# flydog-sdr/FlyDog_SDR_GPS

Measured on NVIDIA B200. Metric: acquisition cells/sec (PRN x Doppler x code-phase), higher is better.
Workload: dtype f32

## Files before the change

flydog_sdr_gps_b200/_build.py:

```python
import os
import shutil
import subprocess

HERE = os.path.dirname(os.path.abspath(__file__))
CSRC = os.path.join(HERE, "csrc")
LIB = os.path.join(CSRC, "libacq_b200.so")
CU_SOURCES = ["acq_kernels.cu", "acq_api.cu", "acq_microbench.cu"]
CPP_SOURCES = ["search_dropin.cpp"]
HEADERS = ["acq_fft.cuh", "acq_geom.h", "acq_kernels.cuh", "e1b_codes.inc", os.path.join("..", "..", "include", "search_dropin.h"),
           os.path.join("..", "..", "include", "acq_b200.h")]

NVCC_FLAGS = ["-gencode", "arch=compute_100a,code=sm_100a", "-lineinfo", "-O3", "-std=c++17",
              "-Xcompiler", "-fPIC", "-shared"]


def _nvcc():
    for cand in (shutil.which("nvcc"), "/usr/local/cuda/bin/nvcc"):
        if cand and os.path.exists(cand):
            return cand
    raise RuntimeError("nvcc not found: cannot build libacq_b200.so")


def needs_build():
    if not os.path.exists(LIB):
        return True
    t = os.path.getmtime(LIB)
    deps = [os.path.join(CSRC, f) for f in CU_SOURCES + CPP_SOURCES + HEADERS]
    return any(os.path.exists(d) and os.path.getmtime(d) > t for d in deps)


def build(force=False, verbose=False, defines=(), out=None):
    if out is None and not force and not needs_build():
        return LIB
    lib = out or LIB
    srcs = [os.path.join(CSRC, f) for f in CU_SOURCES + CPP_SOURCES if os.path.exists(os.path.join(CSRC, f))]
    cmd = [_nvcc()] + NVCC_FLAGS + ["-D" + d for d in defines] + (["-Xptxas", "-v"] if verbose else []) + ["-o", lib + ".tmp"] + srcs
    res = subprocess.run(cmd, capture_output=True, text=True)
    if res.returncode != 0:
        raise RuntimeError("nvcc failed:\n%s\n%s" % (" ".join(cmd), res.stderr[-4000:]))
    os.replace(lib + ".tmp", lib)
    if verbose:
        print(res.stderr)
    return lib


VARIANTS = {
    "l1_multi_tw": ["ACQ_VARIANT_L1_MULTI_TW"],
    "l1_mst": ["ACQ_VARIANT_L1_MST"],
    "l1_cta": ["ACQ_FORCE_L1_CTA=1"],
    "l1_dr_all": ["ACQ_DR_MIN_TILES_PER_SM=0"],
    "l1_dr12": ["ACQ_DR_MIN_TILES_PER_SM=12"],
    "l1_nocr": ["ACQ_L1_CR=0"],
    "l1_sp": ["ACQ_VARIANT_L1_SP"],
    "l1_st": ["ACQ_VARIANT_L1_ST"],
    "l1_ldg": ["ACQ_VARIANT_L1_LDG"],
    "l1_x3": ["ACQ_VARIANT_L1_X3"],
    "l1_x3t": ["ACQ_VARIANT_L1_X3", "ACQ_X3_TMA_D"],
    "e1b_ldg": ["ACQ_VARIANT_E1B_LDG", "ACQ_FORCE_E1B_KERNEL=1"],
    "e1b_cta": ["ACQ_FORCE_E1B_KERNEL=1"],
    "e1b_cluster": ["ACQ_FORCE_E1B_KERNEL=2"],
    "trace": ["ACQ_TRACE"],
    "pdl0": ["ACQ_FORCE_PDL=0"],
    "pdl1": ["ACQ_FORCE_PDL=1"],
    "zcin": ["ACQ_ZC_INPUT=1"],
    "static_tiles": ["ACQ_DYN_MIN_ROUNDS=1000000000"],
    "dyn_tiles": ["ACQ_DYN_MIN_ROUNDS=0"],
    "carve0": ["ACQ_CARVEOUT_MAX=0"],
    "argin0": ["ACQ_ARG_INPUT=0"],
    "devrec": ["ACQ_HOST_RECORDS=0"],
}


def variant_path(name):
    return os.path.join(CSRC, "variants", "libacq_b200_%s.so" % name)


def build_variant(name, force=False):
    path = variant_path(name)
    deps = [os.path.join(CSRC, f) for f in CU_SOURCES + CPP_SOURCES + HEADERS + ["acq_variants.cuh"]]
    fresh = os.path.exists(path) and all(os.path.getmtime(d) <= os.path.getmtime(path) for d in deps if os.path.exists(d))
    if fresh and not force:
        return path
    os.makedirs(os.path.dirname(path), exist_ok=True)
    return build(defines=VARIANTS[name], out=path)


if __name__ == "__main__":
    print(build(force=True, verbose=True))
```

flydog_sdr_gps_b200/csrc/acq_fft.cuh:

```cuda
#pragma once

#include <cuda_runtime.h>
#include <stdint.h>

#include "acq_geom.h"

namespace acq {

__constant__ float2 c_cC[4][16];

__device__ __forceinline__ float2 bc(float s) { return make_float2(s, s); }
__device__ __forceinline__ float2 jmul(float2 a) { return make_float2(-a.y, a.x); }
__device__ __forceinline__ float2 cneg(float2 a) { return make_float2(-a.x, -a.y); }
__device__ __forceinline__ float2 cadd(float2 a, float2 b) { return __fadd2_rn(a, b); }
__device__ __forceinline__ float2 csub(float2 a, float2 b) { return __fadd2_rn(a, cneg(b)); }
__device__ __forceinline__ float2 cadd_jb(float2 a, float2 b) { return __fadd2_rn(a, jmul(b)); }
__device__ __forceinline__ float2 csub_jb(float2 a, float2 b) { return __fadd2_rn(a, cneg(jmul(b))); }
__device__ __forceinline__ float2 cmul(float2 a, float2 w)
{
    return __ffma2_rn(jmul(a), bc(w.y), __fmul2_rn(a, bc(w.x)));
}
__device__ __forceinline__ float2 cfma(float2 a, float2 w, float2 c)
{
    return __ffma2_rn(jmul(a), bc(w.y), __ffma2_rn(a, bc(w.x), c));
// ... 422 lines not shown
    tmem_wait_ld();
    b = TW_AT(15);
    __syncwarp();
    if constexpr (SWZ128) {
        {
            const uint32_t wb = smem_u32(row + c);
            asm volatile("st.shared.v2.f32 [%0], {%1, %2};" ::"r"(wb), "f"(x[r16(0)].x), "f"(x[r16(0)].y) : "memory");
#pragma unroll
            for (int i = 0; i < 15; i++) {
                const int n1 = i + 1;
                const float2 v = cmul(x[r16(n1)], TW_AT(i));
                asm volatile("st.shared.v2.f32 [%0], {%1, %2};" ::"r"((wb ^ (16u * (n1 & 7))) + 128u * n1), "f"(v.x), "f"(v.y) : "memory");
            }
        }
        __syncwarp();
        {
            const uint32_t rb = smem_u32(row + 16 * c + 2 * (c & 7));
#pragma unroll
            for (int j = 0; j < 8; j++)
                asm volatile("ld.shared.v4.f32 {%0, %1, %2, %3}, [%4];"
                             : "=f"(x[2 * j].x), "=f"(x[2 * j].y), "=f"(x[2 * j + 1].x), "=f"(x[2 * j + 1].y)
                             : "r"(rb ^ (16u * j))
                             : "memory");
        }
    } else {
        {
            const uint32_t wb = smem_u32(row + c);
            asm volatile("st.shared.v2.f32 [%0], {%1, %2};" ::"r"(wb), "f"(x[r16(0)].x), "f"(x[r16(0)].y) : "memory");
#pragma unroll
            for (int i = 0; i < 15; i++) {
                const int n1 = i + 1;
                const float2 v = cmul(x[r16(n1)], TW_AT(i));
                asm volatile("st.shared.v2.f32 [%0], {%1, %2};" ::"r"((wb ^ (8u * n1)) + 128u * n1), "f"(v.x), "f"(v.y) : "memory");
            }
        }
        __syncwarp();
        {
            const uint32_t rb = smem_u32(row + 17 * c);
#pragma unroll
            for (int cc = 0; cc < 16; cc++)
                asm volatile("ld.shared.v2.f32 {%0, %1}, [%2];" : "=f"(x[cc].x), "=f"(x[cc].y) : "r"(rb ^ (8u * cc)) : "memory");
        }
    }
    radix16_inv(x);
}
#undef TW_AT

template <bool SWZ128, class PostBarrier>
__device__ __forceinline__ void subfft4096_inv4(float2 (&x)[16], const int k2, float2 &b, float2 *S1b, const int t,
                                                const uint32_t tw_taddr, PostBarrier &&post_barrier)
{
    subfft4096_inv4<SWZ128>(x, k2, b, S1b, t, tw_taddr, [] { __syncthreads(); }, post_barrier);
}

__device__ __forceinline__ void tmem_ld1(uint32_t taddr, float2 &v)
{
    asm volatile("tcgen05.ld.sync.aligned.32x32b.x2.b32 {%0,%1}, [%2];" : "=f"(v.x), "=f"(v.y) : "r"(taddr) : "memory");
}
__device__ __forceinline__ void tmem_st1(uint32_t taddr, const float2 v)
{
    asm volatile("tcgen05.st.sync.aligned.32x32b.x2.b32 [%0], {%1,%2};" ::"r"(taddr), "f"(v.x), "f"(v.y) : "memory");
}

constexpr uint32_t kSwz = ACQ_SWZ128 ? 16u : 8u;
constexpr int kSwzMask = ACQ_SWZ128 ? 7 : 15;

struct BaseFromTmem {
    uint32_t taddr;
    float2 v;
    __device__ __forceinline__ void issue(int k2) { tmem_ld1(taddr + 2 * ((k2 + 1) & 3), v); }
    __device__ __forceinline__ float2 get()
    {
        tmem_wait_ld();
        return v;
    }
};
struct BaseFromGlobal {
    const float2 *bases;
    float2 v;
    __device__ __forceinline__ void issue(int k2) { v = __ldg(bases + 256 * ((k2 + 1) & 3)); }
    __device__ __forceinline__ float2 get() { return v; }
};

template <class BaseSrc, class TeamBarrier, class PostBarrier>
__device__ __forceinline__ void subfft4096_inv4s(float2 (&x)[16], const int k2, float2 &b, float2 *S1b, const int t,
                                                 const float2 *T2s, BaseSrc base_src, TeamBarrier &&team_barrier,
                                                 PostBarrier &&post_barrier)
{
    radix16_inv(x);
    stage_a_store<256>(x, b, S1b + t);
#ifndef ACQ_E1B_TW15
#define ACQ_E1B_TW15 1
#endif
    float2 tw[ACQ_E1B_TW15 ? 15 : 8];
    const float2 *twp = T2s + k2 * (15 * 16) + (t & 15);
#pragma unroll
    for (int i = 0; i < (ACQ_E1B_TW15 ? 15 : 8); i++) tw[i] = twp[i * 16];
    base_src.issue(k2);
    team_barrier();
    post_barrier();
    float2 *row = S1b + (t >> 4) * 256;
    const int c = t & 15;
    {
        const float2 *src = row + c;
#pragma unroll
        for (int bb = 0; bb < 16; bb++) x[bb] = src[16 * bb];
    }
    radix16_inv(x);
    b = base_src.get();
    __syncwarp();
    {
        const uint32_t wb = smem_u32(row + c);
        asm volatile("st.shared.v2.f32 [%0], {%1, %2};" ::"r"(wb), "f"(x[r16(0)].x), "f"(x[r16(0)].y) : "memory");
#pragma unroll
        for (int i = 0; i < 8; i++) {
            const int n1 = i + 1;
            const float2 v = cmul(x[r16(n1)], tw[i]);
            asm volatile("st.shared.v2.f32 [%0], {%1, %2};" ::"r"((wb ^ (kSwz * (n1 & kSwzMask))) + 128u * n1), "f"(v.x), "f"(v.y) : "memory");
        }
#if !ACQ_E1B_TW15
#pragma unroll
        for (int i = 0; i < 7; i++) tw[i] = twp[(i + 8) * 16];
#endif
#pragma unroll
        for (int i = 0; i < 7; i++) {
            const int n1 = i + 9;
            const float2 v = cmul(x[r16(n1)], tw[ACQ_E1B_TW15 ? i + 8 : i]);
            asm volatile("st.shared.v2.f32 [%0], {%1, %2};" ::"r"((wb ^ (kSwz * (n1 & kSwzMask))) + 128u * n1), "f"(v.x), "f"(v.y) : "memory");
        }
    }
    __syncwarp();
#if ACQ_SWZ128
    {
        const uint32_t rb = smem_u32(row + 16 * c + 2 * (c & 7));
#pragma unroll
        for (int j = 0; j < 8; j++)
            asm volatile("ld.shared.v4.f32 {%0, %1, %2, %3}, [%4];"
                         : "=f"(x[2 * j].x), "=f"(x[2 * j].y), "=f"(x[2 * j + 1].x), "=f"(x[2 * j + 1].y)
                         : "r"(rb ^ (16u * j))
                         : "memory");
    }
#else
    {
        const uint32_t rb = smem_u32(row + 17 * c);
#pragma unroll
        for (int cc = 0; cc < 16; cc++)
            asm volatile("ld.shared.v2.f32 {%0, %1}, [%2];" : "=f"(x[cc].x), "=f"(x[cc].y) : "r"(rb ^ (8u * cc)) : "memory");
    }
#endif
    radix16_inv(x);
}
template <class BaseSrc, class PostBarrier>
__device__ __forceinline__ void subfft4096_inv4s(float2 (&x)[16], const int k2, float2 &b, float2 *S1b, const int t,
                                                 const float2 *T2s, BaseSrc base_src, PostBarrier &&post_barrier)
{
    subfft4096_inv4s(x, k2, b, S1b, t, T2s, base_src, [] { __syncthreads(); }, post_barrier);
}

}
```

flydog_sdr_gps_b200/csrc/acq_kernels.cu:

```cuda
#include <cooperative_groups.h>

#include "acq_fft.cuh"
#include "acq_kernels.cuh"

namespace acq {

__constant__ float c_hb[17];

cudaError_t launch_tables_init(const float2 *h_cC, const float *h_hb)
{
    cudaError_t e = cudaMemcpyToSymbol(c_cC, h_cC, sizeof(float2) * 64);
    if (e != cudaSuccess) return e;
    return cudaMemcpyToSymbol(c_hb, h_hb, sizeof(float) * 17);
}

struct HbAcc {
    float re, im;
    __device__ __forceinline__ void first(float xr, float xi, float c)
    {
        re = __fmul_rn(xr, c);
        im = __fmul_rn(xi, c);
    }
    __device__ __forceinline__ void add(float xr, float xi, float c)
    {
// ... 1095 lines not shown
#pragma unroll kMultiUnroll
            for (int k2 = 0; k2 < 4; k2++) {
                float2 *S1b = s.S1 + (it & 1) * kSub;
                const float2 *Dk = S1b + t;
                if (b == 0) {
                    const int r = (k2 - ti.dop) & 3;
                    const int q = (k2 - ti.dop - r) >> 2;
                    const float2 *Ek = s.E + ((p.Q + q) & 1) + t;
                    mbar_wait(bar, (uint32_t)(it & 1));
#pragma unroll
                    for (int a = 0; a < 16; a++) x[a] = Ek[256 * a];
                    tmem_st16(e_taddr + 32 * k2, x);
                    tmem_wait_st();
                } else {
                    tmem_ld16(e_taddr + 32 * k2, x);
                    mbar_wait(bar, (uint32_t)(it & 1));
                    tmem_wait_ld();
                }
#pragma unroll
                for (int a = 0; a < 16; a++) x[a] = cmul_conj_a(Dk[256 * a], x[a]);
                subfft4096_inv4s(x, k2, bw, S1b, t, s.T2, BaseFromGlobal{bases}, [&]() {
                    if (t == 0) {
                        if (b == 0 && k2 == 0) nxt = claim_tile(p, nxt);
                        if (b == p.K - 1 && k2 == 2) publish_tile(feed, p, nxt);
                        if (k2 < 3) issue(ti, b, k2 + 1, (it + 1) & 1);
                        else if (b + 1 < p.K) issue(ti, b + 1, 0, (it + 1) & 1);
                        else {
                            TileIdx tn;
                            if (next_tile(feed, tn)) issue(tn, 0, 0, (it + 1) & 1);
                        }
                    }
                });
                it++;
                if (t == 0 && b == 0 && k2 == 0 && pend_cap >= 0) flush();
                if (k2 == 0) {
#pragma unroll
                    for (int n2 = 0; n2 < 16; n2++) acc[n2] = x[r16(n2)];
                } else {
#pragma unroll
                    for (int n2 = 0; n2 < 16; n2++) acc[n2] = cfma(x[r16(n2)], c_cC[k2][n2], acc[n2]);
                }
            }
#pragma unroll
            for (int n2 = 0; n2 < 16; n2++) P[n2] = (b == 0) ? cpower(acc[n2]) : (P[n2] + cpower(acc[n2]));
        }
        warp_reduce_peak(thread_peak_l1(P, t), red_f + 16 * par, red_i + 8 * par, t);
        pend_cap = ti.cap;
        pend_slot = ti.slot;
        pend_d = ti.d;
        par ^= 1;
        if (!next_tile(feed, ti)) break;
    }
    __syncthreads();
    if (t == 0 && pend_cap >= 0) flush();
    claims_done(p, t);
    search_cta_epilogue(p, t);
    ACQ_TRACE_STAMP(kTrSearchL1, 2);
    tmem_free_cta<2 * kTwCols>(tmem_base, t);
}

#ifndef ACQ_CK_BIG
#define ACQ_CK_BIG 16
#endif
#ifndef ACQ_CK_MID
#define ACQ_CK_MID 4
#endif
constexpr unsigned kCkBig = ACQ_CK_BIG, kCkMid = ACQ_CK_MID;
__device__ __forceinline__ bool chunk_of(const SearchArgs &p, unsigned c, unsigned &start, unsigned &len)
{
    if (c < p.ck_n16) {
        start = kCkBig * c, len = kCkBig;
        return true;
    }
    c -= p.ck_n16;
    if (c < p.ck_n4) {
        start = kCkBig * p.ck_n16 + kCkMid * c, len = kCkMid;
        return true;
    }
    c -= p.ck_n4;
    start = kCkBig * p.ck_n16 + kCkMid * p.ck_n4 + c, len = 1u;
    return start < (unsigned)p.n_tiles;
}

#ifndef ACQ_CR_UNROLL
#define ACQ_CR_UNROLL 4
#endif
template <class PA>
__global__ void __launch_bounds__(256, 2) k_search_l1_cr(const PA p)
{
    extern __shared__ __align__(1024) unsigned char smem[];
    L1MultiSmem s;
    s.S1 = reinterpret_cast<float2 *>(smem);
    s.E = s.S1 + 2 * kSub;
    s.bar = reinterpret_cast<unsigned long long *>(s.E + kEBufElems);
    s.T2 = reinterpret_cast<float2 *>(s.bar + 2);
    s.red_f = reinterpret_cast<float *>(s.T2 + kT2Elems);
    s.red_i = reinterpret_cast<int *>(s.red_f + 32);
    float *red_f = s.red_f;
    int *red_i = s.red_i;
    const int t = threadIdx.x;
    ACQ_TRACE_STAMP(kTrSearchL1, 0);
    constexpr int L = ACQ_LAGS_L1;
    const uint32_t tmem_base = tmem_alloc_cta<2 * kTwCols>(reinterpret_cast<uint32_t *>(red_f + 48), t);
    const uint32_t d_taddr = tmem_base + tmem_lane_base(t) + (uint32_t)((t >> 7) * kTwCols);
    {
        const float4 *src = reinterpret_cast<const float4 *>(p.tables);
        float4 *dst = reinterpret_cast<float4 *>(s.T2);
        for (int i = t; i < kT2Elems / 2; i += 256) dst[i] = __ldg(src + i);
    }
    const float2 *bases = p.tables + kT2Elems + t;
    float2 bw = __ldg(bases);
    const uint32_t bar = smem_u32(s.bar);
    if (t == 0) mbar_init(bar, 1);
    __syncthreads();
    if (p.wait_prior) pdl_wait();
    ACQ_TRACE_STAMP(kTrSearchL1, 1);
    pdl_trigger_search();
    auto issue = [&](const TileIdx &tn, bool fresh_n, int k2n, int half) {
        const int r = (k2n - tn.dop) & 3;
        const int q = (k2n - tn.dop - r) >> 2;
        const float2 *Ek = p.Ep + (size_t)(tn.sat * 4 + r) * p.ext_len + ((p.Q + q) & ~1);
        fence_proxy_async();
        mbar_expect_tx(bar, (uint32_t)(sizeof(float2) * (kEBufElems + (fresh_n ? kSub : 0))));
        tma_load_1d(smem_u32(s.E), Ek, (uint32_t)(sizeof(float2) * kEBufElems), bar);
        if (fresh_n) {
            const float2 *Dk = p.Dp + d_row(p, tn, 0) * kN + k2n * kSub;
            tma_load_1d(smem_u32(s.S1 + half * kSub), Dk, (uint32_t)(sizeof(float2) * kSub), bar);
        }
    };
    int *feed = red_i + 20;
    unsigned cur, left;
    chunk_of(p, blockIdx.x, cur, left);
    left -= 1;
    TileIdx ti(p, cur);
    bool fresh = true;
    unsigned nxt_chunk = blockIdx.x;
    if (t == 0) issue(ti, true, 0, 0);
    int it = 0;
    int par = 0, pend_cap = -1, pend_slot = 0, pend_d = 0;
    auto flush = [&]() {
        store_cell(p, pend_cap, pend_slot, pend_d, merge_warp_peaks(red_f + 16 * (par ^ 1), red_i + 8 * (par ^ 1)), L);
    };

    for (;;) {
        float P[16];
        float2 acc[16];
        float2 x[16];
        constexpr int kCrUnroll = PA::kAided ? 2 : ACQ_CR_UNROLL;
#pragma unroll kCrUnroll
        for (int k2 = 0; k2 < 4; k2++) {
            float2 *S1b = s.S1 + (it & 1) * kSub;
            const int r = (k2 - ti.dop) & 3;
            const int q = (k2 - ti.dop - r) >> 2;
            const float2 *Ek = s.E + ((p.Q + q) & 1) + t;
            if (fresh) {
                const float2 *Dk = S1b + t;
                mbar_wait(bar, (uint32_t)(it & 1));
#pragma unroll
                for (int a = 0; a < 16; a++) x[a] = Dk[256 * a];
                tmem_st16(d_taddr + 32 * k2, x);
                tmem_wait_st();
            } else {
                tmem_ld16(d_taddr + 32 * k2, x);
                mbar_wait(bar, (uint32_t)(it & 1));
                tmem_wait_ld();
            }
#pragma unroll
            for (int a = 0; a < 16; a++) x[a] = cmul_conj_a(x[a], Ek[256 * a]);
            subfft4096_inv4s(x, k2, bw, S1b, t, s.T2, BaseFromGlobal{bases}, [&]() {
                if (t == 0) {
                    if (k2 == 0 && left == 0) nxt_chunk = p.tile_ctr ? gridDim.x + atomicAdd(p.tile_ctr, 1u) : nxt_chunk + gridDim.x;
                    if (k2 == 2) {
                        unsigned ntile = cur + 1, nleft = left - 1;
                        bool valid = true;
                        if (left == 0) {
                            valid = chunk_of(p, nxt_chunk, ntile, nleft);
                            nleft -= 1;
                        }
                        publish_tile(feed, p, valid ? ntile : kNoTile);
                        feed[8] = valid && feed[3] != ti.cap;
                        feed[9] = (int)nleft;
                        feed[10] = (int)ntile;
                    }
                    if (k2 < 3) issue(ti, fresh, k2 + 1, (it + 1) & 1);
                    else {
                        TileIdx tn;
                        if (next_tile(feed, tn)) issue(tn, feed[8] != 0, 0, (it + 1) & 1);
                    }
                }
            });
            it++;
            if (t == 0 && k2 == 0 && pend_cap >= 0) flush();
            if (k2 == 0) {
#pragma unroll
                for (int n2 = 0; n2 < 16; n2++) acc[n2] = x[r16(n2)];
            } else {
#pragma unroll
                for (int n2 = 0; n2 < 16; n2++) acc[n2] = cfma(x[r16(n2)], c_cC[k2][n2], acc[n2]);
            }
        }
#pragma unroll
        for (int n2 = 0; n2 < 16; n2++) P[n2] = cpower(acc[n2]);
        warp_reduce_peak_redux(thread_peak_l1(P, t), red_f + 16 * par, red_i + 8 * par, t);
        pend_cap = ti.cap;
        pend_slot = ti.slot;
        pend_d = ti.d;
        par ^= 1;
        if (!next_tile(feed, ti)) break;
        fresh = feed[8] != 0;
        left = (unsigned)feed[9];
        cur = (unsigned)feed[10];
    }
    __syncthreads();
    if (t == 0 && pend_cap >= 0) flush();
    claims_done(p, t);
    search_cta_epilogue(p, t);
    ACQ_TRACE_STAMP(kTrSearchL1, 2);
    tmem_free_cta<2 * kTwCols>(tmem_base, t);
}

constexpr int kE1bTmemCols = 256;

#ifndef ACQ_E1B_BEST4
#define ACQ_E1B_BEST4 1
#endif
constexpr int kE1bBaseCol = 96;
#ifndef ACQ_E1B_K2_UNROLL
#define ACQ_E1B_K2_UNROLL 4
#endif
constexpr int kE1bK2Unroll = ACQ_E1B_K2_UNROLL;
struct E1bSmem {
    float2 *S1;
    float2 *E;
    unsigned long long *bar;
    float2 *T2;
    float *red_f;
    int *red_i;
};
__host__ __device__ constexpr size_t e1b_smem_bytes()
{
    return sizeof(float2) * (size_t)(2 * kSub + kEBufElems) + 16 + sizeof(float2) * kT2Elems + 64 * sizeof(float);
}
__device__ __forceinline__ E1bSmem e1b_smem_carve(unsigned char *base)
{
    E1bSmem s;
    s.S1 = reinterpret_cast<float2 *>(base);
    s.E = s.S1 + 2 * kSub;
    s.bar = reinterpret_cast<unsigned long long *>(s.E + kEBufElems);
    s.T2 = reinterpret_cast<float2 *>(s.bar + 2);
    s.red_f = reinterpret_cast<float *>(s.T2 + kT2Elems);
    s.red_i = reinterpret_cast<int *>(s.red_f + 32);
    return s;
}

template <class PA>
__global__ void __launch_bounds__(256, 2) k_search_e1b(const PA p)
{
    extern __shared__ __align__(1024) unsigned char smem[];
    const E1bSmem s = e1b_smem_carve(smem);
    float *red_f = s.red_f;
    int *red_i = s.red_i;
    const int t = threadIdx.x;
    constexpr int L = ACQ_LAGS_E1B;
    ACQ_TRACE_STAMP(kTrSearchE1b, 0);
    const uint32_t tmem_base = tmem_alloc_cta<kE1bTmemCols>(reinterpret_cast<uint32_t *>(red_f + 48), t);
    {
        const float4 *src = reinterpret_cast<const float4 *>(p.tables);
        float4 *dst = reinterpret_cast<float4 *>(s.T2);
        for (int i = t; i < kT2Elems / 2; i += 256) dst[i] = __ldg(src + i);
    }
    const uint32_t zaddr = tmem_base + tmem_lane_base(t) + (uint32_t)((t >> 7) * 128);
    float2 bw = __ldg(p.tables + kT2Elems + t);
    tmem_st1(zaddr + kE1bBaseCol, bw);
#pragma unroll
    for (int k2 = 1; k2 < 4; k2++) tmem_st1(zaddr + kE1bBaseCol + 2 * k2, __ldg(p.tables + kT2Elems + k2 * 256 + t));
    tmem_wait_st();
    const uint32_t bar = smem_u32(s.bar);
    if (t == 0) mbar_init(bar, 1);
    __syncthreads();
    if (p.wait_prior) pdl_wait();
    ACQ_TRACE_STAMP(kTrSearchE1b, 1);
    pdl_trigger_search();
    auto issue = [&](const TileIdx &tn, int k2n, int half) {
        const int r = (k2n - tn.dop) & 3;
        const int q = (k2n - tn.dop - r) >> 2;
        const float2 *Dk = p.Dp + d_row(p, tn, 0) * kN + k2n * kSub;
        const float2 *Ek = p.Ep + (size_t)(tn.sat * 4 + r) * p.ext_len + ((p.Q + q) & ~1);
        fence_proxy_async();
        mbar_expect_tx(bar, (uint32_t)(sizeof(float2) * (kSub + kEBufElems)));
        tma_load_1d(smem_u32(s.E), Ek, (uint32_t)(sizeof(float2) * kEBufElems), bar);
        tma_load_1d(smem_u32(s.S1 + half * kSub), Dk, (uint32_t)(sizeof(float2) * kSub), bar);
    };
    TileIdx ti(p, blockIdx.x);
    if (t == 0) issue(ti, 0, 0);
    int *feed = red_i + 20;
    unsigned nxt = blockIdx.x;
    int it = 0;
// ... 520 lines not shown
        for (int j = 0; j < 5; j++) {
#pragma unroll
            for (int off = 16; off > 0; off >>= 1) {
                acc[j].x += __shfl_xor_sync(0xffffffffu, acc[j].x, off);
                acc[j].y += __shfl_xor_sync(0xffffffffu, acc[j].y, off);
            }
        }
        __syncthreads();
        if ((t & 31) == 0) {
#pragma unroll
            for (int j = 0; j < 5; j++) {
                red[t >> 5][2 * j] = acc[j].x;
                red[t >> 5][2 * j + 1] = acc[j].y;
            }
        }
        __syncthreads();
        if (t == 0) {
            float2 R[5];
#pragma unroll
            for (int j = 0; j < 5; j++) {
                R[j] = make_float2(0.0f, 0.0f);
                for (int w = 0; w < 8; w++) R[j].x += red[w][2 * j], R[j].y += red[w][2 * j + 1];
            }
            float sn, cs;
            sincospif((float)((n + 16 * b + cshift) & (kN - 1)) * (1.0f / 8192.0f), &sn, &cs);
            const float2 Xm = cmul(R[0], make_float2(cs, sn)), Xp = cmul(R[4], make_float2(cs, -sn)), X0 = R[2];
            const float2 a = csub(Xm, Xp);
            const float2 g = csub(csub(cadd(X0, X0), Xm), Xp);
            num += a.x * g.x + a.y * g.y;
            den += g.x * g.x + g.y * g.y;
            early += R[1].x * R[2].x + R[1].y * R[2].y;
            late += R[3].x * R[2].x + R[3].y * R[2].y;
            peak += R[2].x * R[2].x + R[2].y * R[2].y;
        }
    }
    if (t == 0) {
        float delta = den > 0.0f ? num / den : 0.0f;
        delta = fminf(1.0f, fmaxf(-1.0f, delta));
        float eps = (early + late) > 0.0f ? (e1b ? (1.0f / 3.0f) : 3.0f) * (late - early) / (early + late) : 0.0f;
        eps = fminf(1.0f, fmaxf(-1.0f, eps));
        const int L = e1b ? ACQ_LAGS_E1B : ACQ_LAGS_L1;
        acq_fine o;
        o.dop_hz = ((p.half_bin ? 0.5f * (float)rc.dop : (float)rc.dop) + delta) * (float)ACQ_BIN_HZ;
        o.code_fs = (float)ACQ_DECIM * ((float)n + eps);
        o.peak = peak;
        int cs = (int)lrintf(o.code_fs) % (L * ACQ_DECIM);
        if (cs < 0) cs += L * ACQ_DECIM;
        o.ca_shift = cs;
        p.out[row] = o;
    }
}

template <class... KArgs, class... Args>
static void launch_k(void (*kern)(KArgs...), dim3 grid, dim3 block, size_t smem, cudaStream_t st, bool pdl, Args... args)
{
    cudaLaunchConfig_t cfg = {};
    cfg.gridDim = grid;
    cfg.blockDim = block;
    cfg.dynamicSmemBytes = smem;
    cfg.stream = st;
    cudaLaunchAttribute at[1];
    at[0].id = cudaLaunchAttributeProgrammaticStreamSerialization;
    at[0].val.programmaticStreamSerializationAllowed = 1;
    cfg.attrs = at;
    cfg.numAttrs = pdl ? 1 : 0;
    cudaLaunchKernelEx(&cfg, kern, KArgs(args)...);
}

static size_t search_l1_smem_bytes() { return fft_smem4_bytes() + 64 * sizeof(float); }
static size_t search_e1b_smem_bytes() { return e1b_smem_bytes(); }
static size_t search_e1b_cluster_smem_bytes() { return fft_smem3_bytes() + 2 * sizeof(float2) * kSub + 64 * sizeof(float); }
static size_t fwd_smem_bytes() { return fft_smem3_bytes() + kZBytes; }

#ifndef ACQ_CARVEOUT_MAX
#define ACQ_CARVEOUT_MAX 1
#endif

static cudaError_t aided_kernels_configure()
{
    using A = AidedSearchArgs;
    const void *k[] = {(const void *)k_search_l1<false, A>, (const void *)k_search_l1_multi<A>, (const void *)k_search_l1_cr<A>,
                       (const void *)k_search_e1b<A>, (const void *)k_search_e1b_multi<A>, (const void *)k_search_e1b_cluster<false, A>,
                       (const void *)k_search_e1b_cluster<true, A>};
    const int smem[] = {(int)search_l1_smem_bytes(), (int)l1_multi_smem_bytes(), (int)l1_multi_smem_bytes(), (int)search_e1b_smem_bytes(),
                        (int)e1b_multi_smem_bytes(), (int)search_e1b_cluster_smem_bytes(), (int)search_e1b_cluster_smem_bytes()};
    cudaError_t e;
    for (int i = 0; i < 7; i++) {
        if ((e = cudaFuncSetAttribute(k[i], cudaFuncAttributeMaxDynamicSharedMemorySize, smem[i]))) return e;
#if ACQ_CARVEOUT_MAX
        if ((e = cudaFuncSetAttribute(k[i], cudaFuncAttributePreferredSharedMemoryCarveout, cudaSharedmemCarveoutMaxShared))) return e;
#endif
    }
    return cudaSuccess;
}

cudaError_t search_kernels_configure()
{
    using S = SearchArgs;
    cudaError_t e;
    const int l1 = (int)search_l1_smem_bytes(), e1 = (int)search_e1b_smem_bytes(), fw = (int)fwd_smem_bytes();
    if ((e = cudaFuncSetAttribute(k_search_l1<false, S>, cudaFuncAttributeMaxDynamicSharedMemorySize, l1))) return e;
#if ACQ_DR_MIN_TILES_PER_SM >= 0
    if ((e = cudaFuncSetAttribute(k_search_l1_dr, cudaFuncAttributeMaxDynamicSharedMemorySize, (int)dr_smem_bytes()))) return e;
#endif
#ifdef ACQ_VARIANT_L1_MST
    if ((e = cudaFuncSetAttribute(k_search_l1_mst, cudaFuncAttributeMaxDynamicSharedMemorySize, (int)dr_smem_bytes()))) return e;
#endif
#ifdef ACQ_VARIANT_L1_SP
    if ((e = cudaFuncSetAttribute(k_search_l1_sp, cudaFuncAttributeMaxDynamicSharedMemorySize, (int)sp_smem_bytes()))) return e;
#endif
#ifdef ACQ_VARIANT_L1_ST
    if ((e = cudaFuncSetAttribute(k_search_l1_st, cudaFuncAttributeMaxDynamicSharedMemorySize, (int)st_smem_bytes()))) return e;
#endif
#ifdef ACQ_VARIANT_L1_MULTI_TW
    if ((e = cudaFuncSetAttribute(k_search_l1<true, S>, cudaFuncAttributeMaxDynamicSharedMemorySize, l1))) return e;
#endif
    if ((e = cudaFuncSetAttribute(k_search_l1_multi<S>, cudaFuncAttributeMaxDynamicSharedMemorySize, (int)l1_multi_smem_bytes()))) return e;
    if ((e = cudaFuncSetAttribute(k_search_l1_cr<S>, cudaFuncAttributeMaxDynamicSharedMemorySize, (int)l1_multi_smem_bytes()))) return e;
    if ((e = cudaFuncSetAttribute(k_search_e1b<S>, cudaFuncAttributeMaxDynamicSharedMemorySize, e1))) return e;
    if ((e = cudaFuncSetAttribute(k_search_e1b_multi<S>, cudaFuncAttributeMaxDynamicSharedMemorySize, (int)e1b_multi_smem_bytes()))) return e;
#ifdef ACQ_VARIANT_L1_X3
    const int l1x = (int)search_l1_x3_smem();
    if ((e = cudaFuncSetAttribute(k_search_l1_x3<false>, cudaFuncAttributeMaxDynamicSharedMemorySize, l1x))) return e;
    if ((e = cudaFuncSetAttribute(k_search_l1_x3<true>, cudaFuncAttributeMaxDynamicSharedMemorySize, l1x))) return e;
#endif
#ifdef ACQ_VARIANT_L1_LDG
    const int l1g = (int)(fft_smem3t_bytes() + 64 * sizeof(float));
    if ((e = cudaFuncSetAttribute(k_search_l1_ldg<false>, cudaFuncAttributeMaxDynamicSharedMemorySize, l1g))) return e;
    if ((e = cudaFuncSetAttribute(k_search_l1_ldg<true>, cudaFuncAttributeMaxDynamicSharedMemorySize, l1g))) return e;
#endif
#ifdef ACQ_VARIANT_E1B_LDG
    const int e1g = (int)(fft_smem3_bytes() + 64 * sizeof(float));
    if ((e = cudaFuncSetAttribute(k_search_e1b_ldg, cudaFuncAttributeMaxDynamicSharedMemorySize, e1g))) return e;
#endif
    const int ec = (int)search_e1b_cluster_smem_bytes();
    if ((e = cudaFuncSetAttribute(k_search_e1b_cluster<false, S>, cudaFuncAttributeMaxDynamicSharedMemorySize, ec))) return e;
    if ((e = cudaFuncSetAttribute(k_search_e1b_cluster<true, S>, cudaFuncAttributeMaxDynamicSharedMemorySize, ec))) return e;
    const int fc = (int)(fft_smem3_bytes() + 2 * sizeof(float2) * kSub);
    if ((e = cudaFuncSetAttribute(k_fwd_fft_cluster<true>, cudaFuncAttributeMaxDynamicSharedMemorySize, fc))) return e;
    if ((e = cudaFuncSetAttribute(k_fwd_fft_cluster<false>, cudaFuncAttributeMaxDynamicSharedMemorySize, fc))) return e;
    if ((e = cudaFuncSetAttribute(k_fwd_fft<true>, cudaFuncAttributeMaxDynamicSharedMemorySize, fw))) return e;
    if ((e = cudaFuncSetAttribute(k_fwd_fft<false>, cudaFuncAttributeMaxDynamicSharedMemorySize, fw))) return e;
#if ACQ_CARVEOUT_MAX
    const void *chain[] = {(const void *)k_front_end<false>, (const void *)k_front_end<true>, (const void *)k_front_end_arg,
                           (const void *)k_fwd_fft<true>, (const void *)k_fwd_fft<false>, (const void *)k_fwd_fft_cluster<true>,
                           (const void *)k_fwd_fft_cluster<false>, (const void *)k_search_l1<false, S>,
#ifdef ACQ_VARIANT_L1_MULTI_TW
                           (const void *)k_search_l1<true, S>,
#endif
#if ACQ_DR_MIN_TILES_PER_SM >= 0
                           (const void *)k_search_l1_dr,
#endif
                           (const void *)k_search_l1_cr<S>, (const void *)k_search_l1_multi<S>, (const void *)k_search_e1b<S>,
                           (const void *)k_search_e1b_multi<S>, (const void *)k_search_e1b_cluster<false, S>,
                           (const void *)k_search_e1b_cluster<true, S>, (const void *)k_pick_small, (const void *)k_best_dop};
    for (const void *f : chain)
        if ((e = cudaFuncSetAttribute(f, cudaFuncAttributePreferredSharedMemoryCarveout, cudaSharedmemCarveoutMaxShared))) return e;
#endif
    return aided_kernels_configure();
}

int launch_front_end(const uint8_t *packed, float2 *x2, const float2 *rot, int n_blocks, int nvar, int K, int sample_bits,
                     int n_shift, int smax, cudaStream_t st)
{
    int launched = 0;
    for (int b0 = 0; b0 < n_blocks; b0 += 32768) {
        const int nb = (n_blocks - b0 < 32768) ? (n_blocks - b0) : 32768;
        const dim3 grid(kN / kFeOut, nb);
        if (sample_bits == 2)
            k_front_end<true><<<grid, 256, 0, st>>>(packed + (size_t)b0 * 2 * ACQ_BLOCK_BYTES,
                                                    x2 + (size_t)b0 * nvar * n_shift * kN, rot, nvar, K, b0, n_shift, smax);
        else
            k_front_end<false><<<grid, 256, 0, st>>>(packed + (size_t)b0 * ACQ_BLOCK_BYTES,
                                                     x2 + (size_t)b0 * nvar * n_shift * kN, rot, nvar, K, b0, n_shift, smax);
        launched++;
    }
    return launched;
}

int launch_front_end_arg(const uint8_t *packed_host, float2 *x2, const float2 *rot, int nvar, int n_shift, int smax,
                         cudaStream_t st)
{
    void *args[] = {const_cast<uint8_t *>(packed_host), &x2, &rot, &nvar, &n_shift, &smax};
    cudaLaunchConfig_t cfg = {};
    cfg.gridDim = dim3(kN / kFeOut, 1);
    cfg.blockDim = dim3(256);
    cfg.stream = st;
    if (cudaLaunchKernelExC(&cfg, reinterpret_cast<const void *>(k_front_end_arg), args) != cudaSuccess) return 0;
    return 1;
}

int launch_hb1_code(const uint32_t *chips, const int *codelen_boc, float2 *x1, int n_sats, cudaStream_t st)
{
    k_hb1_code<<<dim3(128, n_sats), 256, 0, st>>>(chips, codelen_boc, x1);
    return 1;
}

int launch_hb2(const float2 *x1, float2 *x2, const float2 *rot, int n_rows, int nvar, int K, cudaStream_t st)
{
    int launched = 0;
    for (int r0 = 0; r0 < n_rows; r0 += 32768) {
// ... 44 lines not shown
    if (K > 1) return kSearchL1Mst;
#endif
    if (K > 1) return kSearchL1Multi;
    if (half_bin || ACQ_FORCE_L1_CTA) return kSearchL1;
    if (kDrMinTilesPerSm >= 0) return n_tiles < (long long)kDrMinTilesPerSm * sm_count ? kSearchL1 : kSearchL1Dr;
    return ACQ_L1_CR ? kSearchL1Cr : kSearchL1;
}

#ifndef ACQ_DYN_MIN_ROUNDS
#define ACQ_DYN_MIN_ROUNDS 6
#endif
bool search_claims_tiles(long long n_tiles, int grid)
{
    return grid > 0 && n_tiles >= (long long)ACQ_DYN_MIN_ROUNDS * grid;
}

void search_chunks(long long n_tiles, int grid, unsigned *n16, unsigned *n4)
{
    *n16 = *n4 = 0;
    if (!search_claims_tiles(n_tiles, grid)) return;
    const long long singles = 2LL * grid, mids = 2LL * kCkMid * grid;
    long long t2 = n_tiles - singles;
    if (t2 < 0) t2 = 0;
    long long t1 = t2 - mids;
    if (t1 < 0) t1 = 0;
    t1 -= t1 % kCkBig;
    *n16 = (unsigned)(t1 / kCkBig);
    *n4 = (unsigned)((t2 - t1) / kCkMid);
}
long long search_chunk_count(long long n_tiles, int grid)
{
    unsigned n16, n4;
    search_chunks(n_tiles, grid, &n16, &n4);
    return (long long)n16 + n4 + (n_tiles - (long long)kCkBig * n16 - (long long)kCkMid * n4);
}

void search_chunk_lengths(int *big, int *mid)
{
    *big = (int)kCkBig;
    *mid = (int)kCkMid;
}

int search_grid_ctas(long long n_tiles, int kind, int sm_count)
{
    if (n_tiles <= 0 || n_tiles > kMaxTilesPerLaunch) return 0;
    if (kind == kSearchL1Cr) {
        const long long chunks = search_chunk_count(n_tiles, 2 * sm_count);
        return (int)(chunks < 2LL * sm_count ? chunks : 2LL * sm_count);
    }
    long long cap = (long long)sm_count * 2;
    if (kind == kSearchE1bCluster) cap = sm_count / 4;
    if (kind == kSearchL1Dr || kind == kSearchL1Mst) cap = sm_count;
#ifdef ACQ_VARIANT_L1_X3
    if (kind == kSearchL1) cap = (long long)sm_count * 3;
#endif
    return (int)(n_tiles < cap ? n_tiles : cap);
}

bool search_aided_supported(int K, int half_bin, long long tiles_l1, long long tiles_e1b, int sm_count)
{
#if defined(ACQ_VARIANT_L1_X3) || defined(ACQ_VARIANT_L1_LDG) || defined(ACQ_VARIANT_L1_MULTI_TW)
    if (tiles_l1 > 0) return false;
#endif
#ifdef ACQ_VARIANT_E1B_LDG
    if (tiles_e1b > 0) return false;
#endif
    (void)tiles_e1b;
    if (tiles_l1 <= 0) return true;
    const int kind = search_kind_l1(K, half_bin, tiles_l1, sm_count);
    return kind == kSearchL1 || kind == kSearchL1Multi || kind == kSearchL1Cr;
}

static int launch_search_aided(const AidedSearchArgs &a, int kind, int grid, bool e1b, int sm_count, cudaStream_t st, bool pdl)
{
    using A = AidedSearchArgs;
    if (e1b) {
        if (a.K > 1) launch_k(k_search_e1b_multi<A>, grid, 256, e1b_multi_smem_bytes(), st, pdl, a);
        else launch_k(k_search_e1b<A>, grid, 256, search_e1b_smem_bytes(), st, pdl, a);
    } else if (a.K > 1) {
        launch_k(k_search_l1_multi<A>, grid, 256, l1_multi_smem_bytes(), st, pdl, a);
    } else if (kind == kSearchL1Cr) {
        AidedSearchArgs c = a;
        search_chunks(c.n_tiles, 2 * sm_count, &c.ck_n16, &c.ck_n4);
        launch_k(k_search_l1_cr<A>, grid, 256, l1_multi_smem_bytes(), st, pdl, c);
    } else {
        launch_k(k_search_l1<false, A>, grid, 256, search_l1_smem_bytes(), st, pdl, a);
    }
    return 1;
}

int launch_search(const SearchArgs &a_in, bool e1b, int sm_count, cudaStream_t st, bool pdl)
{
    const int kind = e1b ? kSearchE1b : search_kind_l1(a_in.K, a_in.half_bin, a_in.n_tiles, sm_count);
    const int grid = search_grid_ctas(a_in.n_tiles, kind, sm_count);
    if (grid <= 0) return 0;
    SearchArgs a = a_in;
    if (!search_claims_tiles(a.n_tiles, grid)) a.tile_ctr = nullptr;
    if (a.dop_center) return launch_search_aided(AidedSearchArgs(a), kind, grid, e1b, sm_count, st, pdl);
    using S = SearchArgs;
    if (e1b) {
#ifdef ACQ_VARIANT_E1B_LDG
        launch_k(k_search_e1b_ldg, grid, 256, fft_smem3_bytes() + 64 * sizeof(float), st, pdl, a);
#else
        if (a.K > 1) launch_k(k_search_e1b_multi<S>, grid, 256, e1b_multi_smem_bytes(), st, pdl, a);
        else launch_k(k_search_e1b<S>, grid, 256, search_e1b_smem_bytes(), st, pdl, a);
#endif
        return 1;
    }
#if defined(ACQ_VARIANT_L1_X3)
    launch_k(a.K > 1 ? k_search_l1_x3<true> : k_search_l1_x3<false>, grid, 256, search_l1_x3_smem(), st, pdl, a);
#elif defined(ACQ_VARIANT_L1_LDG)
    launch_k(a.K > 1 ? k_search_l1_ldg<true> : k_search_l1_ldg<false>, grid, 256, fft_smem3t_bytes() + 64 * sizeof(float), st,
             pdl, a);
#elif defined(ACQ_VARIANT_L1_MULTI_TW)
    launch_k(a.K > 1 ? k_search_l1<true, S> : k_search_l1<false, S>, grid, 256, search_l1_smem_bytes(), st, pdl, a);
#else
#ifdef ACQ_VARIANT_L1_MST
    if (kind == kSearchL1Mst) launch_k(k_search_l1_mst, grid, kStThreads, dr_smem_bytes(), st, pdl, a);
    else
#endif
    if (a.K > 1) launch_k(k_search_l1_multi<S>, grid, 256, l1_multi_smem_bytes(), st, pdl, a);
    else if (kind == kSearchL1Cr) {
        search_chunks(a.n_tiles, 2 * sm_count, &a.ck_n16, &a.ck_n4);
        launch_k(k_search_l1_cr<S>, grid, 256, l1_multi_smem_bytes(), st, pdl, a);
    }
#if defined(ACQ_VARIANT_L1_SP)
    else if (kind == kSearchL1Dr) launch_k(k_search_l1_sp, grid, kSpThreads, sp_smem_bytes(), st, pdl, a);
#elif defined(ACQ_VARIANT_L1_ST)
    else if (kind == kSearchL1Dr) launch_k(k_search_l1_st, grid, kStThreads, st_smem_bytes(), st, pdl, a);
#endif
#if ACQ_DR_MIN_TILES_PER_SM >= 0
    else if (kind == kSearchL1Dr) launch_k(k_search_l1_dr, grid, kStThreads, dr_smem_bytes(), st, pdl, a);
#endif
    else launch_k(k_search_l1<false, S>, grid, 256, search_l1_smem_bytes(), st, pdl, a);
#endif
    return 1;
}

int launch_search_e1b_cluster(const SearchArgs &a, int sm_count, cudaStream_t st, bool pdl)
{
    const int n_clusters = search_grid_ctas(a.n_tiles, kSearchE1bCluster, sm_count);
    if (n_clusters <= 0) return 0;
    if (a.dop_center)
        launch_k(a.K > 1 ? k_search_e1b_cluster<true, AidedSearchArgs> : k_search_e1b_cluster<false, AidedSearchArgs>, 4 * n_clusters,
                 256, search_e1b_cluster_smem_bytes(), st, pdl, AidedSearchArgs(a));
    else
        launch_k(a.K > 1 ? k_search_e1b_cluster<true, SearchArgs> : k_search_e1b_cluster<false, SearchArgs>, 4 * n_clusters, 256,
                 search_e1b_cluster_smem_bytes(), st, pdl, a);
    return 1;
}

int launch_refine(const float2 *Dp, const float2 *Ep, const acq_record *rec, const int *sat_type, acq_fine *out, int n_rows,
                  int n_slots, int K, int nvar, int half_bin, int ext_len, int Q, int n_shift, int smax, int cd_div,
                  cudaStream_t st)
{
    if (n_rows <= 0) return 0;
    RefineArgs a{Dp, Ep, rec, sat_type, out, n_slots, K, nvar, half_bin, ext_len, Q, n_shift, smax, cd_div};
    k_refine<<<n_rows, 256, 0, st>>>(a);
    return 1;
}

#ifdef ACQ_TRACE
}
extern "C" int acq_trace_read(unsigned long long *out, int n)
{
    const int total = acq::kTraceKernels * acq::kTraceCtas * 4;
    if (!out || n < total) return total;
    if (cudaMemcpyFromSymbol(out, acq::g_trace, sizeof(unsigned long long) * total) != cudaSuccess) return -1;
    static unsigned long long zero[acq::kTraceKernels * acq::kTraceCtas * 4];
    cudaMemcpyToSymbol(acq::g_trace, zero, sizeof zero);
    return total;
}
namespace acq {
#endif

int launch_best_dop(const acq_cell *cells, const int *slot_sat, acq_record *out, int n_cap, int n_slots, int n_dop,
                    PickDop pd, cudaStream_t st, bool pdl)
{
    const int n_rows = n_cap * n_slots;
    launch_k(k_best_dop, (n_rows + 3) / 4, 128, 0, st, pdl, cells, slot_sat, out, n_rows, n_slots, n_dop, pd);
    return 1;
}

int launch_pick_small(const acq_cell *cells, const int *slot_sat, acq_record *out, unsigned *ctas_done, unsigned ctas_total,
                      unsigned *host_flag, unsigned epoch, int n_rows, int n_slots, int n_dop, PickDop pd, cudaStream_t st,
                      bool pdl)
{
    launch_k(k_pick_small, 1, 1024, 0, st, pdl, cells, slot_sat, out, ctas_done, ctas_total, host_flag, epoch, n_rows, n_slots,
             n_dop, pd);
    return 1;
}

}
```

Measured before the change: 133.8 billion.

## Load CR replica rows into registers via ldg instead of TMA staging

In the L1 chunked-round search kernel, the default path stops TMA-loading the code-replica (E) buffer into shared memory. Each thread now prefetches its 16 replica values straight into registers with __ldg, split into an early part issued right after the twiddle stores and a late part issued after the accumulate. This takes the E buffer out of the shared-memory footprint and removes the mbarrier wait on E for non-fresh tiles. It also moves per-tile bookkeeping (cur/left/chunk, pending cell) into shared scalars owned by thread 0, and lowers the default unroll to 2. The cost is higher register pressure and L1/L2 traffic for E under a 256x2 launch bound.

```diff
diff --git a/flydog_sdr_gps_b200/_build.py b/flydog_sdr_gps_b200/_build.py
--- a/flydog_sdr_gps_b200/_build.py
+++ b/flydog_sdr_gps_b200/_build.py
@@ -50,6 +50,7 @@
     "l1_cta": ["ACQ_FORCE_L1_CTA=1"],
     "l1_dr_all": ["ACQ_DR_MIN_TILES_PER_SM=0"],
     "l1_dr12": ["ACQ_DR_MIN_TILES_PER_SM=12"],
+    "cr_etma": ["ACQ_CR_E_TMA=1"],
     "l1_nocr": ["ACQ_L1_CR=0"],
     "l1_sp": ["ACQ_VARIANT_L1_SP"],
     "l1_st": ["ACQ_VARIANT_L1_ST"],
diff --git a/flydog_sdr_gps_b200/csrc/acq_fft.cuh b/flydog_sdr_gps_b200/csrc/acq_fft.cuh
--- a/flydog_sdr_gps_b200/csrc/acq_fft.cuh
+++ b/flydog_sdr_gps_b200/csrc/acq_fft.cuh
@@ -528,10 +528,10 @@
     __device__ __forceinline__ float2 get() { return v; }
 };
 
-template <class BaseSrc, class TeamBarrier, class PostBarrier>
+template <class BaseSrc, class TeamBarrier, class PostBarrier, class PostStores>
 __device__ __forceinline__ void subfft4096_inv4s(float2 (&x)[16], const int k2, float2 &b, float2 *S1b, const int t,
                                                  const float2 *T2s, BaseSrc base_src, TeamBarrier &&team_barrier,
-                                                 PostBarrier &&post_barrier)
+                                                 PostBarrier &&post_barrier, PostStores &&post_stores)
 {
     radix16_inv(x);
     stage_a_store<256>(x, b, S1b + t);
@@ -575,6 +575,7 @@
             asm volatile("st.shared.v2.f32 [%0], {%1, %2};" ::"r"((wb ^ (kSwz * (n1 & kSwzMask))) + 128u * n1), "f"(v.x), "f"(v.y) : "memory");
         }
     }
+    post_stores();
     __syncwarp();
 #if ACQ_SWZ128
     {
@@ -596,11 +597,18 @@
 #endif
     radix16_inv(x);
 }
+template <class BaseSrc, class TeamBarrier, class PostBarrier>
+__device__ __forceinline__ void subfft4096_inv4s(float2 (&x)[16], const int k2, float2 &b, float2 *S1b, const int t,
+                                                 const float2 *T2s, BaseSrc base_src, TeamBarrier &&team_barrier,
+                                                 PostBarrier &&post_barrier)
+{
+    subfft4096_inv4s(x, k2, b, S1b, t, T2s, base_src, team_barrier, post_barrier, [] {});
+}
 template <class BaseSrc, class PostBarrier>
 __device__ __forceinline__ void subfft4096_inv4s(float2 (&x)[16], const int k2, float2 &b, float2 *S1b, const int t,
                                                  const float2 *T2s, BaseSrc base_src, PostBarrier &&post_barrier)
 {
-    subfft4096_inv4s(x, k2, b, S1b, t, T2s, base_src, [] { __syncthreads(); }, post_barrier);
-}
-
-}
+    subfft4096_inv4s(x, k2, b, S1b, t, T2s, base_src, [] { __syncthreads(); }, post_barrier, [] {});
+}
+
+}
diff --git a/flydog_sdr_gps_b200/csrc/acq_kernels.cu b/flydog_sdr_gps_b200/csrc/acq_kernels.cu
--- a/flydog_sdr_gps_b200/csrc/acq_kernels.cu
+++ b/flydog_sdr_gps_b200/csrc/acq_kernels.cu
@@ -1201,9 +1201,19 @@
     return start < (unsigned)p.n_tiles;
 }
 
+#ifndef ACQ_CR_E_TMA
+#define ACQ_CR_E_TMA 0
+#endif
 #ifndef ACQ_CR_UNROLL
-#define ACQ_CR_UNROLL 4
-#endif
+#define ACQ_CR_UNROLL (ACQ_CR_E_TMA ? 4 : 2)
+#endif
+#ifndef ACQ_CR_E_EARLY
+#define ACQ_CR_E_EARLY 8
+#endif
+__host__ __device__ constexpr size_t l1_cr_smem_bytes()
+{
+    return l1_multi_smem_bytes() - (ACQ_CR_E_TMA ? 0 : sizeof(float2) * kEBufElems) + 16 * sizeof(int);
+}
 template <class PA>
 __global__ void __launch_bounds__(256, 2) k_search_l1_cr(const PA p)
 {
@@ -1211,7 +1221,7 @@
     L1MultiSmem s;
     s.S1 = reinterpret_cast<float2 *>(smem);
     s.E = s.S1 + 2 * kSub;
-    s.bar = reinterpret_cast<unsigned long long *>(s.E + kEBufElems);
+    s.bar = reinterpret_cast<unsigned long long *>(s.E + (ACQ_CR_E_TMA ? kEBufElems : 0));
     s.T2 = reinterpret_cast<float2 *>(s.bar + 2);
     s.red_f = reinterpret_cast<float *>(s.T2 + kT2Elems);
     s.red_i = reinterpret_cast<int *>(s.red_f + 32);
@@ -1235,30 +1245,61 @@
     if (p.wait_prior) pdl_wait();
     ACQ_TRACE_STAMP(kTrSearchL1, 1);
     pdl_trigger_search();
-    auto issue = [&](const TileIdx &tn, bool fresh_n, int k2n, int half) {
-        const int r = (k2n - tn.dop) & 3;
-        const int q = (k2n - tn.dop - r) >> 2;
-        const float2 *Ek = p.Ep + (size_t)(tn.sat * 4 + r) * p.ext_len + ((p.Q + q) & ~1);
+    int *own = red_i + 32;
+    const float2 **own_d = reinterpret_cast<const float2 **>(own + 6);
+    auto issue = [&](bool fresh_n, int sat_n, int dop_n, int k2n, int half) {
+#if ACQ_CR_E_TMA
+        const int r = (k2n - dop_n) & 3;
+        const int q = (k2n - dop_n - r) >> 2;
+        const float2 *Ek = p.Ep + (size_t)(sat_n * 4 + r) * p.ext_len + ((p.Q + q) & ~1);
         fence_proxy_async();
         mbar_expect_tx(bar, (uint32_t)(sizeof(float2) * (kEBufElems + (fresh_n ? kSub : 0))));
         tma_load_1d(smem_u32(s.E), Ek, (uint32_t)(sizeof(float2) * kEBufElems), bar);
-        if (fresh_n) {
-            const float2 *Dk = p.Dp + d_row(p, tn, 0) * kN + k2n * kSub;
-            tma_load_1d(smem_u32(s.S1 + half * kSub), Dk, (uint32_t)(sizeof(float2) * kSub), bar);
-        }
+#else
+        if (!fresh_n) return;
+        fence_proxy_async();
+        mbar_expect_tx(bar, (uint32_t)(sizeof(float2) * kSub));
+#endif
+        if (fresh_n) tma_load_1d(smem_u32(s.S1 + half * kSub), *own_d + k2n * kSub, (uint32_t)(sizeof(float2) * kSub), bar);
     };
+#if !ACQ_CR_E_TMA
+    float2 e[16];
+    auto load_e = [&](int sat, int dop, int k2n, int a0, int a1) {
+        const int r = (k2n - dop) & 3;
+        const int q = (k2n - dop - r) >> 2;
+        const float2 *Eg = p.Ep + (size_t)(sat * 4 + r) * p.ext_len + p.Q + q + t;
+#pragma unroll
+        for (int a = a0; a < a1; a++) e[a] = __ldg(Eg + 256 * a);
+    };
+#endif
     int *feed = red_i + 20;
-    unsigned cur, left;
-    chunk_of(p, blockIdx.x, cur, left);
-    left -= 1;
-    TileIdx ti(p, cur);
+    int sat, dop;
+    {
+        unsigned cur, left;
+        chunk_of(p, blockIdx.x, cur, left);
+        const TileIdx ti(p, cur);
+        sat = ti.sat, dop = ti.dop;
+        if (t == 0) {
+            own[0] = (int)cur, own[1] = (int)left - 1, own[2] = (int)blockIdx.x, own[3] = -1;
+            own[8] = ti.cap, own[9] = ti.slot, own[10] = ti.d;
+            *own_d = p.Dp + d_row(p, ti, 0) * kN;
+            issue(true, sat, dop, 0, 0);
+        }
+    }
     bool fresh = true;
-    unsigned nxt_chunk = blockIdx.x;
-    if (t == 0) issue(ti, true, 0, 0);
-    int it = 0;
-    int par = 0, pend_cap = -1, pend_slot = 0, pend_d = 0;
+#if !ACQ_CR_E_TMA
+    load_e(sat, dop, 0, 0, 16);
+    auto prefetch_e = [&](int k2, int a0, int a1) {
+        if (k2 < 3) load_e(sat, dop, k2 + 1, a0, a1);
+        else {
+            const bool nx = feed[0] != 0;
+            load_e(nx ? feed[1] : sat, nx ? feed[5] : dop, 0, a0, a1);
+        }
+    };
+#endif
+    int par = 0;
     auto flush = [&]() {
-        store_cell(p, pend_cap, pend_slot, pend_d, merge_warp_peaks(red_f + 16 * (par ^ 1), red_i + 8 * (par ^ 1)), L);
+        store_cell(p, own[3], own[4], own[5], merge_warp_peaks(red_f + 16 * (par ^ 1), red_i + 8 * (par ^ 1)), L);
     };
 
     for (;;) {
@@ -1268,48 +1309,60 @@
         constexpr int kCrUnroll = PA::kAided ? 2 : ACQ_CR_UNROLL;
 #pragma unroll kCrUnroll
         for (int k2 = 0; k2 < 4; k2++) {
-            float2 *S1b = s.S1 + (it & 1) * kSub;
-            const int r = (k2 - ti.dop) & 3;
-            const int q = (k2 - ti.dop - r) >> 2;
-            const float2 *Ek = s.E + ((p.Q + q) & 1) + t;
+            float2 *S1b = s.S1 + (k2 & 1) * kSub;
             if (fresh) {
                 const float2 *Dk = S1b + t;
-                mbar_wait(bar, (uint32_t)(it & 1));
+                mbar_wait(bar, (uint32_t)(k2 & 1));
 #pragma unroll
                 for (int a = 0; a < 16; a++) x[a] = Dk[256 * a];
                 tmem_st16(d_taddr + 32 * k2, x);
                 tmem_wait_st();
             } else {
                 tmem_ld16(d_taddr + 32 * k2, x);
-                mbar_wait(bar, (uint32_t)(it & 1));
+#if ACQ_CR_E_TMA
+                mbar_wait(bar, (uint32_t)(k2 & 1));
+#endif
                 tmem_wait_ld();
             }
+#if ACQ_CR_E_TMA
+            const int r = (k2 - dop) & 3;
+            const int q = (k2 - dop - r) >> 2;
+            const float2 *Ek = s.E + ((p.Q + q) & 1) + t;
 #pragma unroll
             for (int a = 0; a < 16; a++) x[a] = cmul_conj_a(x[a], Ek[256 * a]);
-            subfft4096_inv4s(x, k2, bw, S1b, t, s.T2, BaseFromGlobal{bases}, [&]() {
+#else
+#pragma unroll
+            for (int a = 0; a < 16; a++) x[a] = cmul_conj_a(x[a], e[a]);
+#endif
+            subfft4096_inv4s(x, k2, bw, S1b, t, s.T2, BaseFromGlobal{bases}, [] { __syncthreads(); }, [&]() {
                 if (t == 0) {
-                    if (k2 == 0 && left == 0) nxt_chunk = p.tile_ctr ? gridDim.x + atomicAdd(p.tile_ctr, 1u) : nxt_chunk + gridDim.x;
+                    if (k2 == 0 && own[1] == 0)
+                        own[2] = (int)(p.tile_ctr ? gridDim.x + atomicAdd(p.tile_ctr, 1u) : (unsigned)own[2] + gridDim.x);
                     if (k2 == 2) {
-                        unsigned ntile = cur + 1, nleft = left - 1;
+                        unsigned ntile = (unsigned)own[0] + 1, nleft = (unsigned)own[1] - 1;
                         bool valid = true;
-                        if (left == 0) {
-                            valid = chunk_of(p, nxt_chunk, ntile, nleft);
+                        if (own[1] == 0) {
+                            valid = chunk_of(p, (unsigned)own[2], ntile, nleft);
                             nleft -= 1;
                         }
                         publish_tile(feed, p, valid ? ntile : kNoTile);
-                        feed[8] = valid && feed[3] != ti.cap;
-                        feed[9] = (int)nleft;
-                        feed[10] = (int)ntile;
+                        feed[8] = valid && feed[3] != own[8];
+                        own[0] = (int)ntile, own[1] = (int)nleft;
                     }
-                    if (k2 < 3) issue(ti, fresh, k2 + 1, (it + 1) & 1);
-                    else {
-                        TileIdx tn;
-                        if (next_tile(feed, tn)) issue(tn, feed[8] != 0, 0, (it + 1) & 1);
+                    TileIdx tn;
+                    if (k2 < 3) {
+                        issue(fresh, sat, dop, k2 + 1, (k2 + 1) & 1);
+                    } else if (next_tile(feed, tn)) {
+                        if (feed[8]) *own_d = p.Dp + d_row(p, tn, 0) * kN;
+                        issue(feed[8] != 0, tn.sat, tn.dop, 0, 0);
                     }
                 }
+            }, [&]() {
+#if !ACQ_CR_E_TMA
+                prefetch_e(k2, 0, ACQ_CR_E_EARLY);
+#endif
             });
-            it++;
-            if (t == 0 && k2 == 0 && pend_cap >= 0) flush();
+            if (t == 0 && k2 == 0 && own[3] >= 0) flush();
             if (k2 == 0) {
 #pragma unroll
                 for (int n2 = 0; n2 < 16; n2++) acc[n2] = x[r16(n2)];
@@ -1317,21 +1370,24 @@
 #pragma unroll
                 for (int n2 = 0; n2 < 16; n2++) acc[n2] = cfma(x[r16(n2)], c_cC[k2][n2], acc[n2]);
             }
+#if !ACQ_CR_E_TMA
+            if (ACQ_CR_E_EARLY < 16) prefetch_e(k2, ACQ_CR_E_EARLY, 16);
+#endif
         }
 #pragma unroll
         for (int n2 = 0; n2 < 16; n2++) P[n2] = cpower(acc[n2]);
         warp_reduce_peak_redux(thread_peak_l1(P, t), red_f + 16 * par, red_i + 8 * par, t);
-        pend_cap = ti.cap;
-        pend_slot = ti.slot;
-        pend_d = ti.d;
+        if (t == 0) {
+            own[3] = own[8], own[4] = own[9], own[5] = own[10];
+            own[8] = feed[3], own[9] = feed[2], own[10] = feed[4];
+        }
         par ^= 1;
-        if (!next_tile(feed, ti)) break;
+        if (!feed[0]) break;
+        sat = feed[1], dop = feed[5];
         fresh = feed[8] != 0;
-        left = (unsigned)feed[9];
-        cur = (unsigned)feed[10];
     }
     __syncthreads();
-    if (t == 0 && pend_cap >= 0) flush();
+    if (t == 0 && own[3] >= 0) flush();
     claims_done(p, t);
     search_cta_epilogue(p, t);
     ACQ_TRACE_STAMP(kTrSearchL1, 2);
@@ -2018,7 +2074,7 @@
     const void *k[] = {(const void *)k_search_l1<false, A>, (const void *)k_search_l1_multi<A>, (const void *)k_search_l1_cr<A>,
                        (const void *)k_search_e1b<A>, (const void *)k_search_e1b_multi<A>, (const void *)k_search_e1b_cluster<false, A>,
                        (const void *)k_search_e1b_cluster<true, A>};
-    const int smem[] = {(int)search_l1_smem_bytes(), (int)l1_multi_smem_bytes(), (int)l1_multi_smem_bytes(), (int)search_e1b_smem_bytes(),
+    const int smem[] = {(int)search_l1_smem_bytes(), (int)l1_multi_smem_bytes(), (int)l1_cr_smem_bytes(), (int)search_e1b_smem_bytes(),
                         (int)e1b_multi_smem_bytes(), (int)search_e1b_cluster_smem_bytes(), (int)search_e1b_cluster_smem_bytes()};
     cudaError_t e;
     for (int i = 0; i < 7; i++) {
@@ -2052,7 +2108,7 @@
     if ((e = cudaFuncSetAttribute(k_search_l1<true, S>, cudaFuncAttributeMaxDynamicSharedMemorySize, l1))) return e;
 #endif
     if ((e = cudaFuncSetAttribute(k_search_l1_multi<S>, cudaFuncAttributeMaxDynamicSharedMemorySize, (int)l1_multi_smem_bytes()))) return e;
-    if ((e = cudaFuncSetAttribute(k_search_l1_cr<S>, cudaFuncAttributeMaxDynamicSharedMemorySize, (int)l1_multi_smem_bytes()))) return e;
+    if ((e = cudaFuncSetAttribute(k_search_l1_cr<S>, cudaFuncAttributeMaxDynamicSharedMemorySize, (int)l1_cr_smem_bytes()))) return e;
     if ((e = cudaFuncSetAttribute(k_search_e1b<S>, cudaFuncAttributeMaxDynamicSharedMemorySize, e1))) return e;
     if ((e = cudaFuncSetAttribute(k_search_e1b_multi<S>, cudaFuncAttributeMaxDynamicSharedMemorySize, (int)e1b_multi_smem_bytes()))) return e;
 #ifdef ACQ_VARIANT_L1_X3
@@ -2263,7 +2319,7 @@
     } else if (kind == kSearchL1Cr) {
         AidedSearchArgs c = a;
         search_chunks(c.n_tiles, 2 * sm_count, &c.ck_n16, &c.ck_n4);
-        launch_k(k_search_l1_cr<A>, grid, 256, l1_multi_smem_bytes(), st, pdl, c);
+        launch_k(k_search_l1_cr<A>, grid, 256, l1_cr_smem_bytes(), st, pdl, c);
     } else {
         launch_k(k_search_l1<false, A>, grid, 256, search_l1_smem_bytes(), st, pdl, a);
     }
@@ -2303,7 +2359,7 @@
     if (a.K > 1) launch_k(k_search_l1_multi<S>, grid, 256, l1_multi_smem_bytes(), st, pdl, a);
     else if (kind == kSearchL1Cr) {
         search_chunks(a.n_tiles, 2 * sm_count, &a.ck_n16, &a.ck_n4);
-        launch_k(k_search_l1_cr<S>, grid, 256, l1_multi_smem_bytes(), st, pdl, a);
+        launch_k(k_search_l1_cr<S>, grid, 256, l1_cr_smem_bytes(), st, pdl, a);
     }
 #if defined(ACQ_VARIANT_L1_SP)
     else if (kind == kSearchL1Dr) launch_k(k_search_l1_sp, grid, kSpThreads, sp_smem_bytes(), st, pdl, a);
```

Measured after the change: 122.0 billion (median of 6 runs). 0.911x the previous value.
